# autonomousvision/sdfstudio

Hardware: NVIDIA H100
Metric: rays/sec at 4096 rays x 128 samples (higher is better)
Workload: dtype bf16x3 (fp32 accumulate)

## Files before the change

sdfstudio_b200/csrc/field_tc.h:

```cpp
#pragma once
#include "field_plan.h"

namespace sdfb200 {


constexpr int kEpiWarps = 8;
constexpr int kEpiThreads = kEpiWarps * 32;
constexpr int kTcThreads = kEpiThreads + 128;
constexpr int kEncThreads = 96;
constexpr int kEncItems0 = 288, kEncItems1 = 256, kEncItems2 = 224;
static_assert(kEncItems0 + kEncItems1 + kEncItems2 == 768, "the encoder warps' items cover the tile");
static_assert(kEncItems0 % 32 == 0 && kEncItems1 % 32 == 0, "a warp stages whole 32-row batches (colour_static_tile shuffles across them)");
__host__ __device__ constexpr int enc_item_begin(int w) { return w == 0 ? 0 : w == 1 ? kEncItems0 : w == 2 ? kEncItems0 + kEncItems1 : 768; }
constexpr int kConsumerRegs = 216;
constexpr int kProducerRegs = 72;
static_assert(2 * (kConsumerRegs - 168) <= 168 - kProducerRegs, "setmaxnreg.inc would wait for registers nobody frees");
constexpr int kStages = 5;
constexpr int kKB = 16;
constexpr int kMaxGridDim = 32;
constexpr int kMaxPe = 60;
constexpr int kPeRows = 64;
constexpr int kInK = 96;
constexpr float kHalfPiF = 1.5707963267948966f;
constexpr uint32_t kAPlane = 32 * 2048;
constexpr uint32_t kImgPlane = (kInK / 8) * 128 * 16;
__host__ __device__ constexpr uint32_t tc_stage_bytes(int planes) { return (uint32_t)planes * 256 * kKB * 2; }

enum { PRM_B_G0 = 0, PRM_B_G1, PRM_W_G2 , PRM_B_C0, PRM_B_C1, PRM_W_C2 , kPrmRows = PRM_W_C2 + 3 };
enum { HS_SDF = 0, HS_GRAD , HS_RGB = HS_GRAD + 3 , kHsRows = HS_RGB + 3 };
enum { GEOM_PX = 0, GEOM_PY, GEOM_PZ, GEOM_DX, GEOM_DY, GEOM_DZ, kGeomRows };

struct TcSmem { size_t a, ring, prm, hs, coldesc, hx, bytes; };
__host__ __device__ constexpr TcSmem tc_smem(int planes) {
  TcSmem s{};
  s.ring = s.a + (size_t)planes * kAPlane;
  s.prm = s.ring + (size_t)kStages * tc_stage_bytes(planes);
  s.hs = s.prm + kPrmRows * 256 * 4;
  s.coldesc = s.hs + 2 * kHsRows * 128 * 4;
  s.hx = s.coldesc + 96 * 16;
  s.bytes = s.hx + 128 * 8;
  return s;
}
constexpr size_t kSmemPerBlock = 232448;
constexpr size_t kStaticSmem = 1024;
static_assert(tc_smem(2).bytes + kStaticSmem <= kSmemPerBlock, "shared memory of k_field_tc at two planes");

constexpr size_t kFragWords = 64 * 256;
struct TcScratch { size_t sig, h2, slots, slot_bytes, geo, cs, jpe, jg, geom, ray, bytes; };
__host__ __device__ constexpr TcScratch tc_scratch(int planes) {
  TcScratch s{};
  s.h2 = s.sig + kFragWords * 4;
  s.slots = s.h2 + (size_t)planes * kAPlane;
  s.cs = s.geo + (size_t)planes * kImgPlane;
  s.jpe = s.cs + (size_t)planes * kImgPlane;
  s.jg = s.jpe + (size_t)kPeRows * 128 * 4;
  s.geom = s.jg + (size_t)kMaxGridDim * 3 * 128 * 4;
  s.ray = s.geom + (size_t)kGeomRows * 128 * 4;
  s.slot_bytes = s.ray + 128 * 8;
  s.bytes = s.slots + 2 * s.slot_bytes;
  return s;
}
__host__ __device__ constexpr size_t kScratchPerCta(int planes) { return tc_scratch(planes).bytes; }

__host__ __device__ constexpr int tc_layer_np(int L) { return L == L_B0 ? 128 : 256; }
__host__ __device__ constexpr int tc_layer_k(int L) { return L == L_G0 || L == L_C0MISC ? kInK : 256; }
__host__ __device__ constexpr int tc_layer_kblk(int L) { return kKB * 256 / tc_layer_np(L); }
__host__ __device__ constexpr int tc_layer_nkb(int L) { return tc_layer_k(L) / tc_layer_kblk(L); }
constexpr bool tc_blocks_fill_stages() {
  for (int L = 0; L < L_COUNT; ++L)
    if (tc_layer_np(L) * tc_layer_kblk(L) != 256 * kKB || tc_layer_kblk(L) % 16 != 0 || tc_layer_k(L) % tc_layer_kblk(L) != 0) return false;
  return true;
}
static_assert(tc_blocks_fill_stages(), "every streamed weight block must be one full ring stage of whole K steps");

struct TcLayer {
  unsigned long long w_off;
};

struct TcArgs {
  sdfb200_grid_t grid;
  TcLayer layer[L_COUNT];
  int use_grid, pe_degree, use_pe, contraction, pe_dim, grid_dim, app_dim, use_n_dot_v;
  int mode;
  int n_samples, has_bins, n_tiles;
  long long n_points;
  float rgb_padding, cos_anneal;
  const float *origins, *directions, *bins, *appearance, *variance, *beta, *beta_min;
  const void* table;
  const char* blob;
  unsigned long long b_g0, b_g1, b_g2, w_g2, b_c0, b_c1, w_c2, b_c2;
  char* scratch;
  sdfb200_field_out_t out;
  int render;
  sdfb200_field_render_t rnd;
};

int launch_field_tc_p2_torch(const TcArgs& a, int grid, size_t smem, cudaStream_t st);
int launch_field_tc_p2_tcnn(const TcArgs& a, int grid, size_t smem, cudaStream_t st);
int launch_field_tc_p1_torch(const TcArgs& a, int grid, size_t smem, cudaStream_t st);
int launch_field_tc_p1_tcnn(const TcArgs& a, int grid, size_t smem, cudaStream_t st);

}
```

sdfstudio_b200/csrc/field_tc_kernel.cuh:

```cuda
#pragma once
#include "field_tc.h"
#include "grid.cuh"
#include "tc_common.cuh"

namespace sdfb200 {
using namespace tc;

__device__ __forceinline__ void named_sync(int id, int n) { asm volatile("bar.sync %0, %1;" ::"r"(id), "r"(n) : "memory"); }
constexpr int kEncBar = 3;

__device__ __forceinline__ const float* point_bin(const TcArgs& a, int tile, int row, long long& ray) {
  const long long p0 = (long long)tile * 128;
  const long long ray0 = p0 / a.n_samples;
  const int s = (int)(p0 - ray0 * a.n_samples) + (int)(min(p0 + row, a.n_points - 1) - p0);
  ray = ray0 + s / a.n_samples;
  return a.bins + ray * (a.n_samples + 1) + s % a.n_samples;
}

struct PointGeom { float px, py, pz, dx, dy, dz, delta, t0, t1; long long ray; };
__device__ __forceinline__ PointGeom point_geom(const TcArgs& a, int tile, int row) {
  const long long p = min((long long)tile * 128 + row, a.n_points - 1);
  PointGeom g;
  g.dx = g.dy = g.dz = 0.f; g.delta = 0.f; g.t0 = g.t1 = 0.f;
  g.ray = p;
  if (a.has_bins) {
    const float* bin = point_bin(a, tile, row, g.ray);
    const float t0 = __ldg(bin);
    g.t0 = t0;
    g.t1 = __ldg(bin + 1);
    g.delta = __fsub_rn(g.t1, t0);
    g.dx = __ldg(a.directions + g.ray * 3); g.dy = __ldg(a.directions + g.ray * 3 + 1); g.dz = __ldg(a.directions + g.ray * 3 + 2);
    g.px = __fadd_rn(__ldg(a.origins + g.ray * 3 + 0), __fmul_rn(g.dx, t0));
    g.py = __fadd_rn(__ldg(a.origins + g.ray * 3 + 1), __fmul_rn(g.dy, t0));
    g.pz = __fadd_rn(__ldg(a.origins + g.ray * 3 + 2), __fmul_rn(g.dz, t0));
  } else {
    g.px = __ldg(a.origins + p * 3); g.py = __ldg(a.origins + p * 3 + 1); g.pz = __ldg(a.origins + p * 3 + 2);
    if (a.directions) { g.dx = __ldg(a.directions + p * 3); g.dy = __ldg(a.directions + p * 3 + 1); g.dz = __ldg(a.directions + p * 3 + 2); }
  }
  if (a.contraction != SDFB200_CONTRACT_NONE) {
    const float mag = a.contraction == SDFB200_CONTRACT_LINF
                          ? fmaxf(fabsf(g.px), fmaxf(fabsf(g.py), fabsf(g.pz)))
                          : sqrtf(__fadd_rn(__fadd_rn(__fmul_rn(g.px, g.px), __fmul_rn(g.py, g.py)), __fmul_rn(g.pz, g.pz)));
    if (mag >= 1.f) {
      const float k = __fsub_rn(2.f, __fdiv_rn(1.f, mag));
      g.px = __fmul_rn(k, __fdiv_rn(g.px, mag)); g.py = __fmul_rn(k, __fdiv_rn(g.py, mag)); g.pz = __fmul_rn(k, __fdiv_rn(g.pz, mag));
    }
  }
  return g;
}

static __device__ __forceinline__ void sincos_call(float x, float* s, float* c) { sincosf(x, s, c); }
static __device__ __forceinline__ float sin_call(float x) { return sinf(x); }

template <int P>
struct Slot {
  uint8_t* base;
  __device__ __forceinline__ Slot(char* slots, uint32_t s) : base(reinterpret_cast<uint8_t*>(slots) + s * tc_scratch(P).slot_bytes) {}
  __device__ __forceinline__ uint8_t* geo() const { return base + tc_scratch(P).geo; }
  __device__ __forceinline__ uint8_t* cs() const { return base + tc_scratch(P).cs; }
  __device__ __forceinline__ float* jpe() const { return reinterpret_cast<float*>(base + tc_scratch(P).jpe); }
  __device__ __forceinline__ float* jg() const { return reinterpret_cast<float*>(base + tc_scratch(P).jg); }
  __device__ __forceinline__ float (*geom() const)[128] { return reinterpret_cast<float (*)[128]>(base + tc_scratch(P).geom); }
  __device__ __forceinline__ long long* ray() const { return reinterpret_cast<long long*>(base + tc_scratch(P).ray); }
};

template <int P>
__device__ __forceinline__ void stage_geom(const TcArgs& a, int tile, int et, const Slot<P>& s) {
  float (*gm)[128] = s.geom();
#pragma unroll 1
  for (int row = et; row < 128; row += kEncThreads) {
    const PointGeom g = point_geom(a, tile, row);
    gm[GEOM_PX][row] = g.px; gm[GEOM_PY][row] = g.py; gm[GEOM_PZ][row] = g.pz;
    gm[GEOM_DX][row] = g.dx; gm[GEOM_DY][row] = g.dy; gm[GEOM_DZ][row] = g.dz;
    s.ray()[row] = g.ray;
  }
}

template <int P, int LAYOUT>
__device__ __forceinline__ void encode_tile_grid(const TcArgs& a, int row, int grp, const Slot<P>& s, uint64_t pol_table) {
  const float (*gm)[128] = s.geom();
  float* Jg = s.jg();
  const float x01 = (gm[GEOM_PX][row] + 2.0f) * 0.25f, y01 = (gm[GEOM_PY][row] + 2.0f) * 0.25f, z01 = (gm[GEOM_PZ][row] + 2.0f) * 0.25f;
  const int l_end = min(4 * grp + 4, min(a.grid.n_levels, a.grid.active_levels));
  if (a.use_grid && a.mode != 0) {
#pragma unroll 1
    for (int l = 4 * grp; l < l_end; ++l) {
      LevelCtx c;
      level_prepare<LAYOUT>(a.grid, l, x01, y01, z01, c);
      if (a.grid.table_dtype == SDFB200_DT_F16) level_prefetch_l2<__half, 2>(a.table, c);
      else level_prefetch_l2<float, 2>(a.table, c);
    }
  }
  uint32_t h0 = 0u, h1 = 0u, h2 = 0u, h3 = 0u, l0 = 0u, l1 = 0u, l2 = 0u, l3 = 0u;
#pragma unroll 1
  for (int l = 4 * grp; l < 4 * grp + 4; ++l) {
    float o[2] = {0.f, 0.f};
    float dj[2][3] = {{0.f, 0.f, 0.f}, {0.f, 0.f, 0.f}};
    if (a.use_grid && l < l_end) {
      LevelCtx c;
      float tv[8][2];
      level_prepare<LAYOUT>(a.grid, l, x01, y01, z01, c);
      if (a.grid.table_dtype == SDFB200_DT_F16) level_fetch<__half, 2, true>(a.table, c, tv, pol_table);
      else level_fetch<float, 2, true>(a.table, c, tv, pol_table);
      level_finish<2, LAYOUT>(a.grid, c, tv, o, dj);
    }
    uint32_t hi, lo;
    split2(o[0], o[1], hi, lo);
    h0 = h1; h1 = h2; h2 = h3; h3 = hi;
    l0 = l1; l1 = l2; l2 = l3; l3 = lo;
    if (a.mode != 0 && l < a.grid.n_levels) {
#pragma unroll
      for (int f = 0; f < 2; ++f) {
        const int cg = l * 2 + f;
        Jg[(cg * 3 + 0) * 128 + row] = 0.25f * dj[f][0];
        Jg[(cg * 3 + 1) * 128 + row] = 0.25f * dj[f][1];
        Jg[(cg * 3 + 2) * 128 + row] = 0.25f * dj[f][2];
      }
    }
  }
  store_a_chunk<P>(s.geo(), kImgPlane, row, grp, make_uint4(h0, h1, h2, h3), make_uint4(l0, l1, l2, l3));
}

template <int P>
__device__ __forceinline__ void encode_tile_pe(const TcArgs& a, int tile, int row, const Slot<P>& s) {
  const long long p = (long long)tile * 128 + row;
  const float (*gm)[128] = s.geom();
  const float px = gm[GEOM_PX][row], py = gm[GEOM_PY][row], pz = gm[GEOM_PZ][row];
  if (p < a.n_points) {
    if (a.out.points_norm) a.out.points_norm[p] = sqrtf(__fadd_rn(__fadd_rn(__fmul_rn(px, px), __fmul_rn(py, py)), __fmul_rn(pz, pz)));
    if (a.out.points) { a.out.points[p * 3] = px; a.out.points[p * 3 + 1] = py; a.out.points[p * 3 + 2] = pz; }
  }
  const int deg = a.pe_degree, half = 3 * deg;
  uint8_t* img = s.geo();
  float* Jpe = s.jpe();
  const uint4 z4 = make_uint4(0u, 0u, 0u, 0u);
#pragma unroll 1
  for (int ch = 4; ch < kInK / 8; ++ch) store_a_chunk<P>(img, kImgPlane, row, ch, z4, z4);
#pragma unroll 1
  for (int i = 0; i < a.pe_dim; ++i) {
    const int ia = i >= half ? i - half : i;
    const int b = ia / deg, k = ia - b * deg;
    const float fr = (float)(1 << k);
    const float xb = b == 0 ? px : (b == 1 ? py : pz);
    const float arg = i >= half ? xb * fr + kHalfPiF : xb * fr;
    float sv, cv;
    sincos_call(arg, &sv, &cv);
    store_a<P>(img, kImgPlane, row, 32 + i, a.use_pe ? sv : 0.f);
    if (a.mode != 0) Jpe[i * 128 + row] = a.use_pe ? fr * cv : 0.f;
  }
  store_a<P>(img, kImgPlane, row, 32 + a.pe_dim + 0, px);
  store_a<P>(img, kImgPlane, row, 32 + a.pe_dim + 1, py);
  store_a<P>(img, kImgPlane, row, 32 + a.pe_dim + 2, pz);
}

__device__ __forceinline__ float dir_enc(float dx, float dy, float dz, int k) {
  const int i = k < 12 ? k : k - 12, b = i >> 2;
  const float db = b == 0 ? dx : (b == 1 ? dy : dz);
  const float arg = db * (float)(1 << (i & 3));
  return sin_call(k < 12 ? arg : arg + kHalfPiF);
}

template <int P>
__device__ __forceinline__ void colour_static_tile(const TcArgs& a, int row, const Slot<P>& s) {
  const float (*gm)[128] = s.geom();
  const float px = gm[GEOM_PX][row], py = gm[GEOM_PY][row], pz = gm[GEOM_PZ][row];
  const float dx = gm[GEOM_DX][row], dy = gm[GEOM_DY][row], dz = gm[GEOM_DZ][row];
  const long long ray = s.ray()[row];
  const bool one_ray = __match_any_sync(0xffffffffu, ray) == 0xffffffffu;
  const int lane = row & 31;
  const float own = one_ray && lane < 24 ? dir_enc(dx, dy, dz, lane) : 0.f;
  uint8_t* img = s.cs();
  const uint4 z4 = make_uint4(0u, 0u, 0u, 0u);
#pragma unroll 1
  for (int ch = 1; ch < kInK / 8; ++ch) store_a_chunk<P>(img, kImgPlane, row, ch, z4, z4);
  store_a<P>(img, kImgPlane, row, 8 + 0, px); store_a<P>(img, kImgPlane, row, 8 + 1, py); store_a<P>(img, kImgPlane, row, 8 + 2, pz);
#pragma unroll 1
  for (int k = 0; k < 24; ++k) {
    const float shared = __shfl_sync(0xffffffffu, own, k);
    store_a<P>(img, kImgPlane, row, 8 + 3 + k, one_ray ? shared : dir_enc(dx, dy, dz, k));
  }
  store_a<P>(img, kImgPlane, row, 8 + 27, dx); store_a<P>(img, kImgPlane, row, 8 + 28, dy); store_a<P>(img, kImgPlane, row, 8 + 29, dz);
  if (a.appearance != nullptr) {
#pragma unroll 1
    for (int j = 0; j < a.app_dim; ++j) store_a<P>(img, kImgPlane, row, 8 + 30 + j, __ldg(a.appearance + ray * a.app_dim + j));
  }
}

#ifdef SDFB200_TC_TIMING
__device__ long long g_tc_timing[16 * 48];
#define TC_PUT(tno, k, v)                                                                                            \
  do {                                                                                                               \
    if (blockIdx.x == 0 && (tno) >= 0 && (tno) < 16) g_tc_timing[(tno) * 48 + (k)] = (v);                            \
  } while (0)
#else
#define TC_PUT(tno, k, v) do { (void)(v); } while (0)
#endif
#define TC_STAMP(k) do { if (tid == 0) TC_PUT(tile_no, k, TC_CLOCK()); } while (0)

struct TcBars {
  Handoff<kStages> ring;
  Handoff<2> enc;
  Handoff<1> a;
  Handoff<2> hs;
  uint64_t cop[2][2];
};

template <int P>
__device__ __forceinline__ void produce_all(const TcArgs& a, int nlayers, uint8_t* abuf, uint8_t* ring, char* slots, TcBars& b) {
  uint32_t j = 0;
  int tile_no = 0;
  for (int tile = blockIdx.x; tile < a.n_tiles; tile += gridDim.x, ++tile_no) {
    long long waited = 0;
    b.a.wait_empty(tile_no);
    b.enc.wait_full(tile_no);
    const uint8_t* geo = Slot<P>(slots, b.enc.slot(tile_no)).geo();
    mbar_arrive_expect_tx(b.a.full_bar(tile_no), (uint32_t)P * kImgPlane);
#pragma unroll
    for (int pl = 0; pl < P; ++pl) bulk_g2s(abuf + pl * kAPlane, geo + pl * kImgPlane, kImgPlane, b.a.full_bar(tile_no));
    for (int L = 0; L < nlayers; ++L) {
      for (int kb = 0; kb < tc_layer_nkb(L); ++kb, ++j)
        ring_fill(b.ring, ring, j, reinterpret_cast<const uint8_t*>(a.blob) + a.layer[L].w_off, kb, tc_stage_bytes(P), &waited);
    }
    TC_PUT(tile_no, 10, waited);
  }
}

constexpr int kH2Early = 32 - kInK / 8;
template <int P, int L>
__device__ __forceinline__ void layer_mma(float (&acc)[4][32], bool zero, uint32_t a_base, const uint8_t* ring, Handoff<kStages>& rb, uint32_t& it,
                                          int lane, long long& waited, uint64_t* h2_late, uint32_t h2_parity) {
  constexpr int N = tc_layer_np(L);
  constexpr int KSTEPS = tc_layer_kblk(L) / 16;
  constexpr uint32_t lbo_b = N * 16, plane_b = N * KSTEPS * 16 * 2;
  float (&d)[N / 2] = *reinterpret_cast<float (*)[N / 2]>(&acc[0][0]);
  if (zero) {
#pragma unroll
    for (int i = 0; i < N / 2; ++i) d[i] = 0.f;
  }
#pragma unroll 1
  for (int kb = 0; kb < tc_layer_nkb(L); ++kb, ++it) {
    if (L == L_C0H && kb * KSTEPS == kH2Early / 2) mbar_wait(h2_late, h2_parity);
    rb.wait_full(it, &waited);
    const uint32_t wbase = smem_u32(ring + (size_t)rb.slot(it) * tc_stage_bytes(P));
    wg_fence_acc(d);
    wg_arrive();
#pragma unroll
    for (int j = 0; j < KSTEPS; ++j) {
      const int kstep = kb * KSTEPS + j;
      const int ka = L == L_C0H ? (kstep + kInK / 16) % 16 : kstep;
      wgmma_kstep_wide_ss<P, N>(d, a_desc(a_base, ka), a_desc(a_base + kAPlane, ka), wbase + j * 2 * lbo_b, plane_b, lbo_b);
    }
    wg_commit();
    wg_wait<0>();
    wg_fence_acc(d);
    __syncwarp();
    if (lane == 0) rb.arrive_empty(it);
  }
}

struct TileCtx {
  const TcArgs& a;
  int tid, t, wg, wrow0;
  int r0, cq;
  uint8_t* abuf;
  const float (*prm)[256];
  float (*hs)[128];
  const float4* coldesc;
  float sdf_bias;
  uint32_t* sig_s;
  uint8_t* h2img;
  char* slots;
  __device__ __forceinline__ int unit(int c, int i) const { return (c * 16 + (i >> 1)) * kEpiThreads + tid; }
};

__device__ __forceinline__ uint32_t unorm16x2_encode(float s0, float s1) {
  const float f0 = __fadd_rn(__fmul_rn(s0, 65535.0f), 12582912.0f), f1 = __fadd_rn(__fmul_rn(s1, 65535.0f), 12582912.0f);
  return __byte_perm(__float_as_uint(f0), __float_as_uint(f1), 0x5410);
}
__device__ __forceinline__ float unorm16_lo(uint32_t w) { return __fsub_rn(__uint_as_float(__byte_perm(w, 0x4B00u, 0x5410)), 8388608.0f) * (1.0f / 65535.0f); }
__device__ __forceinline__ float unorm16_hi(uint32_t w) { return __fsub_rn(__uint_as_float(__byte_perm(w, 0x4B00u, 0x5432)), 8388608.0f) * (1.0f / 65535.0f); }

__device__ __forceinline__ void acc_shift(float (&acc)[4][32]) {
#pragma unroll
  for (int c = 0; c < 3; ++c) {
#pragma unroll
    for (int i = 0; i < 32; ++i) acc[c][i] = acc[c + 1][i];
  }
}

template <int N>
__device__ __forceinline__ void load_prm_block(const float* prow, int cq, int c, int j0, float2 (&v)[N]) {
#pragma unroll
  for (int j = 0; j < N; ++j) v[j] = *reinterpret_cast<const float2*>(prow + frag_col(cq, c, 4 * (j0 + j)));
}

template <int P>
__device__ __forceinline__ void epi_e0(const TileCtx& x, float (&acc)[4][32]) {
  const float* p_bg0 = x.prm[PRM_B_G0];
#pragma unroll 1
  for (int c = 0; c < 4; ++c, acc_shift(acc)) {
    float2 bias[8];
    load_prm_block(p_bg0, x.cq, c, 0, bias);
#pragma unroll
    for (int i = 0; i < 32; i += 2) {
      const int col = frag_col(x.cq, c, i), row = frag_row(x.r0, i);
      const float2 b2 = bias[i >> 2];
      float h0, h1, s0, s1;
      softplus100_fast(acc[0][i] + b2.x, h0, s0);
      softplus100_fast(acc[0][i + 1] + b2.y, h1, s1);
      store_a_pair<P>(x.abuf, kAPlane, row, col, h0, h1);
      if (x.a.mode != 0) x.sig_s[x.unit(c, i)] = unorm16x2_encode(s0, s1);
    }
  }
}

template <int P>
__device__ __forceinline__ void epi_e1(const TileCtx& x, int tile, float (&acc)[4][32]) {
  const TcArgs& a = x.a;
  const float* p_bg1 = x.prm[PRM_B_G1];
  const float* p_wg2 = x.prm[PRM_W_G2];
  float sp0 = 0.f, sp1 = 0.f;
#pragma unroll 1
  for (int c = 0; c < 4; ++c, acc_shift(acc)) {
    float2 bias[2], wrow[2];
#pragma unroll
    for (int i = 0; i < 32; i += 2) {
      if (i % 8 == 0) { load_prm_block(p_bg1, x.cq, c, i >> 2, bias); load_prm_block(p_wg2, x.cq, c, i >> 2, wrow); }
      const int col = frag_col(x.cq, c, i), row = frag_row(x.r0, i);
      const float2 b2 = bias[(i >> 2) & 1];
      const float2 w2 = wrow[(i >> 2) & 1];
      float h0, h1, s0, s1;
      softplus100_fast(acc[0][i] + b2.x, h0, s0);
      softplus100_fast(acc[0][i + 1] + b2.y, h1, s1);
      float& sp = frag_half(i) ? sp1 : sp0;
      sp = fmaf(w2.x, h0, sp);
      sp = fmaf(w2.y, h1, sp);
      if (a.mode != 0) {
        store_a_pair<P>(x.h2img, kAPlane, row, col, h0, h1);
        store_a_pair<P>(x.abuf, kAPlane, row, col, w2.x * s0, w2.y * s1);
      }
    }
  }
  if (a.mode != 0) fence_async_global();
  sp0 = quad_sum(sp0);
  sp1 = quad_sum(sp1);
  if ((x.t & 3) < 2) {
    const int h = x.t & 1, row = x.r0 + 8 * h;
    const float sdf = (h ? sp1 : sp0) + x.sdf_bias;
    const long long p = (long long)tile * 128 + row;
    if (p < a.n_points && a.out.sdf) a.out.sdf[p] = sdf;
    if (a.mode != 0) x.hs[HS_SDF][row] = sdf;
  }
}

template <int P>
__device__ __forceinline__ void epi_eb1(const TileCtx& x, float (&acc)[4][32]) {
  uint32_t sw[16], sw_next[16];
#pragma unroll
  for (int k = 0; k < 16; ++k) sw[k] = x.sig_s[x.unit(0, 2 * k)];
#pragma unroll 1
  for (int c = 0; c < 4; ++c, acc_shift(acc)) {
    if (c < 3) {
#pragma unroll
      for (int k = 0; k < 16; ++k) sw_next[k] = x.sig_s[x.unit(c + 1, 2 * k)];
    }
#pragma unroll
    for (int i = 0; i < 32; i += 2) {
      const int col = frag_col(x.cq, c, i), row = frag_row(x.r0, i);
      const uint32_t w = sw[i >> 1];
      store_a_pair<P>(x.abuf, kAPlane, row, col, acc[0][i] * unorm16_lo(w), acc[0][i + 1] * unorm16_hi(w));
    }
    if (c < 3) {
#pragma unroll
      for (int k = 0; k < 16; ++k) sw[k] = sw_next[k];
    }
  }
}

__device__ __forceinline__ float4 col_desc(const TcArgs& a, int ip) {
  const int deg = a.pe_degree, half = 3 * deg;
  int jrow = -1, ax = -1;
  if (ip < a.pe_dim) {
    const int ia = ip >= half ? ip - half : ip;
    ax = ia < deg ? 0 : (ia < 2 * deg ? 1 : 2);
    jrow = ip * 128;
  } else if (ip - a.pe_dim < 3) {
    ax = ip - a.pe_dim;
  }
  return make_float4(__int_as_float(jrow), ax == 0 ? 1.f : 0.f, ax == 1 ? 1.f : 0.f, ax == 2 ? 1.f : 0.f);
}

template <int P>
__device__ __forceinline__ void copy_chunks(uint8_t* abuf, int a_chunk, const uint8_t* src, uint32_t src_plane, int src_chunk, int n, int wrow0,
                                            uint64_t* bar, int lane) {
  for (int k0 = 0; k0 < P * n; k0 += 32) {
    const int k = k0 + lane;
    if (k < P * n) {
      const int pl = k / n, c = k - pl * n;
      bulk_g2s(abuf + pl * kAPlane + (a_chunk + c) * kAChunk + wrow0 * 16, src + pl * src_plane + (src_chunk + c) * kAChunk + wrow0 * 16, 64 * 16, bar);
    }
  }
}
template <int P>
__device__ __forceinline__ void colour_copy(const TileCtx& x, bool early, const uint8_t* cs, uint64_t* bar) {
  constexpr int kMisc = kInK / 8;
  const int lane = x.t & 31;
  if (lane == 0) mbar_arrive_expect_tx(bar, (uint32_t)P * (early ? (kMisc - 1) + kH2Early : 32 - kH2Early) * 64 * 16);
  __syncwarp();
  if (early) {
    copy_chunks<P>(x.abuf, 1, cs, kImgPlane, 1, kMisc - 1, x.wrow0, bar, lane);
    copy_chunks<P>(x.abuf, kMisc, x.h2img, kAPlane, 0, kH2Early, x.wrow0, bar, lane);
  } else {
    copy_chunks<P>(x.abuf, 0, x.h2img, kAPlane, kH2Early, 32 - kH2Early, x.wrow0, bar, lane);
  }
}

template <int P>
__device__ __forceinline__ void epi_eb0(const TileCtx& x, const Slot<P>& s, const float (&acc)[4][32]) {
  const TcArgs& a = x.a;
  const float* Jpe = s.jpe();
  const float* Jg = s.jg();
  float g0x = 0.f, g0y = 0.f, g0z = 0.f, g1x = 0.f, g1y = 0.f, g1z = 0.f;
#pragma unroll
  for (int c = 0; c < 2; ++c) {
#pragma unroll
    for (int i = 0; i < 32; ++i) {
      const int col = frag_col(x.cq, c, i), row = frag_row(x.r0, i);
      const bool h = frag_half(i);
      float& gx = h ? g1x : g0x;
      float& gy = h ? g1y : g0y;
      float& gz = h ? g1z : g0z;
      const float g = acc[c][i];
      if (c == 0 && i < 16) {
        const bool live = col < a.grid_dim;
        const float* j = Jg + col * 3 * 128 + row;
        const float jx = live ? j[0] : 0.f, jy = live ? j[128] : 0.f, jz = live ? j[256] : 0.f;
        gx = fmaf(g, jx, gx); gy = fmaf(g, jy, gy); gz = fmaf(g, jz, gz);
      } else {
        const float4 d = x.coldesc[col - 32];
        const int jrow = __float_as_int(d.x);
        const float tv = __fmul_rn(g, jrow >= 0 ? Jpe[jrow + row] : 1.f);
        gx = fmaf(tv, d.y, gx); gy = fmaf(tv, d.z, gy); gz = fmaf(tv, d.w, gz);
      }
    }
  }
  g0x = quad_sum(g0x); g0y = quad_sum(g0y); g0z = quad_sum(g0z);
  g1x = quad_sum(g1x); g1y = quad_sum(g1y); g1z = quad_sum(g1z);
  if ((x.t & 3) < 2) {
    const int h = x.t & 1, row = x.r0 + 8 * h;
    const float (*gm)[128] = s.geom();
    const float grx = h ? g1x : g0x, gry = h ? g1y : g0y, grz = h ? g1z : g0z;
    const float3 n = normalize_eps(grx, gry, grz);
    const float c0v[8] = {grx, gry, grz, a.use_n_dot_v ? n.x * gm[GEOM_DX][row] + n.y * gm[GEOM_DY][row] + n.z * gm[GEOM_DZ][row] : 0.f,
                          0.f, 0.f, 0.f, 0.f};
    store_a_chunk<P>(x.abuf, kAPlane, row, 0, c0v);
    x.hs[HS_GRAD][row] = grx; x.hs[HS_GRAD + 1][row] = gry; x.hs[HS_GRAD + 2][row] = grz;
  }
}

template <int P>
__device__ __forceinline__ void epi_ec0(const TileCtx& x, float (&acc)[4][32]) {
  const float* p_bc0 = x.prm[PRM_B_C0];
#pragma unroll 1
  for (int c = 0; c < 4; ++c, acc_shift(acc)) {
    float2 bias[8];
    load_prm_block(p_bc0, x.cq, c, 0, bias);
#pragma unroll
    for (int i = 0; i < 32; i += 2) {
      const int col = frag_col(x.cq, c, i), row = frag_row(x.r0, i);
      const float2 b2 = bias[i >> 2];
      store_a_pair<P>(x.abuf, kAPlane, row, col, fmaxf(acc[0][i] + b2.x, 0.f), fmaxf(acc[0][i + 1] + b2.y, 0.f));
    }
  }
}

__device__ __forceinline__ void epi_ec1(const TileCtx& x, float (&acc)[4][32]) {
  const float* p_bc1 = x.prm[PRM_B_C1];
  const float (*p_wc2)[256] = x.prm + PRM_W_C2;
  float r0r = 0.f, r0g = 0.f, r0b = 0.f, r1r = 0.f, r1g = 0.f, r1b = 0.f;
#pragma unroll 1
  for (int c = 0; c < 4; ++c, acc_shift(acc)) {
#pragma unroll
    for (int i = 0; i < 32; ++i) {
      const int col = frag_col(x.cq, c, i);
      const bool h = frag_half(i);
      float& rr = h ? r1r : r0r;
      float& rg = h ? r1g : r0g;
      float& rb = h ? r1b : r0b;
      const float v = fmaxf(acc[0][i] + p_bc1[col], 0.f);
      rr = fmaf(p_wc2[0][col], v, rr);
      rg = fmaf(p_wc2[1][col], v, rg);
      rb = fmaf(p_wc2[2][col], v, rb);
    }
  }
  r0r = quad_sum(r0r); r0g = quad_sum(r0g); r0b = quad_sum(r0b);
  r1r = quad_sum(r1r); r1g = quad_sum(r1g); r1b = quad_sum(r1b);
  if ((x.t & 3) < 2) {
    const int h = x.t & 1, row = x.r0 + 8 * h;
    x.hs[HS_RGB][row] = h ? r1r : r0r; x.hs[HS_RGB + 1][row] = h ? r1g : r0g; x.hs[HS_RGB + 2][row] = h ? r1b : r0b;
  }
}

struct HeadsXfer { double wtot[2][4]; float csum[2][4][8]; };
static_assert(sizeof(TcBars) + sizeof(HeadsXfer) <= kStaticSmem, "static shared memory of k_field_tc (kStaticSmem)");
enum { HR_ALPHA = HS_SDF , HR_NORMAL = HS_GRAD , HR_RGB = HS_RGB  };
struct RayEnd { int q; double tot; float last[3]; };
struct HeadsClock { long long rows, scan, sums; };

__device__ __forceinline__ float sample_mid(const TcArgs& a, int tile, int row) {
  if (!a.has_bins) return 0.f;
  long long ray;
  const float* b = point_bin(a, tile, row, ray);
  return __fdiv_rn(__fadd_rn(__ldg(b), __ldg(b + 1)), 2.0f);
}

__device__ __forceinline__ void heads_rows(const TcArgs& a, float (*hs)[128], double* hx, double* wtot, int tile, int q, int lane,
                                           float& dmin, float& dmax, HeadsClock& clk) {
  long long tc0 = TC_CLOCK();
  const float* b_c2 = reinterpret_cast<const float*>(a.blob + a.b_c2);
  const int row = q * 32 + lane;
  const long long p_raw = (long long)tile * 128 + row;
  const bool valid = p_raw < a.n_points;
  const long long p = valid ? p_raw : a.n_points - 1;
  const PointGeom pg = point_geom(a, tile, row);
  const float dirx = pg.dx, diry = pg.dy, dirz = pg.dz, delta = pg.delta;
  const float sdf = hs[HS_SDF][row], grx = hs[HS_GRAD][row], gry = hs[HS_GRAD + 1][row], grz = hs[HS_GRAD + 2][row];
  const float3 nv = normalize_eps(grx, gry, grz);
  const float nx = nv.x, ny = nv.y, nz = nv.z;
  float rgbv[3];
#pragma unroll
  for (int c = 0; c < 3; ++c) rgbv[c] = padded_rgb(sigmoidf_(hs[HS_RGB + c][row] + __ldg(b_c2 + c)), a.rgb_padding);
  float density = 0.f, alpha = 0.f;
  if (a.out.density || (a.render && a.rnd.from_density)) density = sdf_density(sdf, __ldg(a.beta), __ldg(a.beta_min));
  if (a.out.alpha || (a.render && !a.rnd.from_density))
    alpha = neus_alpha(sdf, dirx * grx + diry * gry + dirz * grz, delta, __ldg(a.variance), a.cos_anneal);
  if (valid) {
    if (a.out.rgb) { a.out.rgb[p * 3] = rgbv[0]; a.out.rgb[p * 3 + 1] = rgbv[1]; a.out.rgb[p * 3 + 2] = rgbv[2]; }
    if (a.out.gradients) { a.out.gradients[p * 3] = grx; a.out.gradients[p * 3 + 1] = gry; a.out.gradients[p * 3 + 2] = grz; }
    if (a.out.normals) { a.out.normals[p * 3] = nx; a.out.normals[p * 3 + 1] = ny; a.out.normals[p * 3 + 2] = nz; }
    if (a.out.density) a.out.density[p] = density;
    if (a.out.occupancy) a.out.occupancy[p] = occupancy(sdf);
    if (a.out.alpha) a.out.alpha[p] = alpha;
  }
  { const long long c = TC_CLOCK(); clk.rows += c - tc0; tc0 = c; }
  if (!a.render) return;
  const int S = a.n_samples;
  const int s_idx = row % S;
  const bool dens = a.rnd.from_density != 0;
  const float dd = valid ? __fmul_rn(delta, density) : 0.f;
  double f = dens ? (double)dd : (valid ? (double)neus_trans_factor(alpha) : 1.0);
  double incl = f;
#pragma unroll
  for (int d = 1; d < 32; d <<= 1) {
    const double o = __shfl_up_sync(0xffffffffu, incl, d);
    if (lane >= d && s_idx >= d) incl = dens ? incl + o : incl * o;
  }
  double excl = __shfl_up_sync(0xffffffffu, incl, 1);
  if (lane == 0 || s_idx == 0) excl = dens ? 0.0 : 1.0;
  const float al = dens ? __fsub_rn(1.0f, expf(-dd)) : alpha;
  const float mid = __fdiv_rn(__fadd_rn(pg.t0, pg.t1), 2.0f);
  if (valid) { dmin = fminf(dmin, mid); dmax = fmaxf(dmax, mid); }
  if (S > 32) {
    if (lane == 31) wtot[q] = incl;
    hx[row] = excl;
    hs[HR_ALPHA][row] = al;
    hs[HR_NORMAL][row] = nx; hs[HR_NORMAL + 1][row] = ny; hs[HR_NORMAL + 2][row] = nz;
    hs[HR_RGB][row] = rgbv[0]; hs[HR_RGB + 1][row] = rgbv[1]; hs[HR_RGB + 2][row] = rgbv[2];
    clk.scan += TC_CLOCK() - tc0;
    return;
  }
  const float T = dens ? expf(-(float)excl) : (float)excl;
  const float w = valid ? __fmul_rn(al, T) : 0.f;
  if (valid && a.rnd.weights) a.rnd.weights[p] = w;
  { const long long c = TC_CLOCK(); clk.scan += c - tc0; tc0 = c; }
  float vs[8] = {w, w * rgbv[0], w * rgbv[1], w * rgbv[2], w * nx, w * ny, w * nz, w * mid};
#pragma unroll
  for (int d = 1; d < 32; d <<= 1) {
    if (d < S) {
#pragma unroll
      for (int k = 0; k < 8; ++k) vs[k] += __shfl_down_sync(0xffffffffu, vs[k], d);
    }
  }
  const int last = (lane - s_idx) + S - 1;
  const double tot = __shfl_sync(0xffffffffu, dens ? excl : incl, last);
  const float lc[3] = {__shfl_sync(0xffffffffu, rgbv[0], last), __shfl_sync(0xffffffffu, rgbv[1], last), __shfl_sync(0xffffffffu, rgbv[2], last)};
  const long long ray = (long long)tile * (128 / S) + row / S;
  if (s_idx == 0 && ray * S < a.n_points) {
    finish_ray(ray, vs[0], {vs[1], vs[2], vs[3]}, {vs[4], vs[5], vs[6]}, vs[7], a.rnd.bg_mode, a.rnd.bg, lc, a.rnd.clamp01, a.rnd.out.rgb,
               a.rnd.out.accumulation, a.rnd.out.normal, a.rnd.out.depth);
    if (a.rnd.bg_transmittance) a.rnd.bg_transmittance[ray] = dens ? expf(-(float)tot) : (float)tot;
  }
  clk.sums += TC_CLOCK() - tc0;
}

__device__ __forceinline__ void composite_chunk(const TcArgs& a, const float (*hs)[128], const double* hx, const double* wtot, float (*csum)[8],
                                                int tile, int q, int lane, RayEnd& end, HeadsClock& clk) {
  long long tc0 = TC_CLOCK();
  const int row = q * 32 + lane;
  const long long p_raw = (long long)tile * 128 + row;
  const bool valid = p_raw < a.n_points;
  const long long p = valid ? p_raw : a.n_points - 1;
  const int S = a.n_samples;
  const bool dens = a.rnd.from_density != 0;
  const int first = (q * 32 / S) * (S / 32);
  double excl = hx[row];
  for (int w2 = first; w2 < q; ++w2) excl = dens ? excl + wtot[w2] : excl * wtot[w2];
  const float T = dens ? expf(-(float)excl) : (float)excl;
  const float w = valid ? __fmul_rn(hs[HR_ALPHA][row], T) : 0.f;
  if (valid && a.rnd.weights) a.rnd.weights[p] = w;
  { const long long c = TC_CLOCK(); clk.scan += c - tc0; tc0 = c; }
  const float rgbv[3] = {hs[HR_RGB][row], hs[HR_RGB + 1][row], hs[HR_RGB + 2][row]};
  float vs[8] = {w, w * rgbv[0], w * rgbv[1], w * rgbv[2], w * hs[HR_NORMAL][row], w * hs[HR_NORMAL + 1][row], w * hs[HR_NORMAL + 2][row],
                 w * sample_mid(a, tile, row)};
#pragma unroll
  for (int d = 1; d < 32; d <<= 1) {
#pragma unroll
    for (int k = 0; k < 8; ++k) vs[k] += __shfl_down_sync(0xffffffffu, vs[k], d);
  }
  if (lane == 0) {
#pragma unroll
    for (int k = 0; k < 8; ++k) csum[q][k] = vs[k];
  }
  if (q == first + S / 32 - 1) {
    end.q = q;
    if (dens) {
      end.tot = __shfl_sync(0xffffffffu, excl, 31);
    } else {
      end.tot = 1.0;
      for (int w2 = first; w2 <= q; ++w2) end.tot *= wtot[w2];
    }
#pragma unroll
    for (int c = 0; c < 3; ++c) end.last[c] = __shfl_sync(0xffffffffu, rgbv[c], 31);
  }
  clk.sums += TC_CLOCK() - tc0;
}

__device__ __forceinline__ void finish_rays(const TcArgs& a, const float (*csum)[8], int tile, int lane, const RayEnd& end, HeadsClock& clk) {
  const long long tc0 = TC_CLOCK();
  const int S = a.n_samples;
  const long long ray = (long long)tile * (128 / S) + end.q * 32 / S;
  if (end.q >= 0 && lane == 0 && ray * S < a.n_points) {
    float s[8] = {0.f, 0.f, 0.f, 0.f, 0.f, 0.f, 0.f, 0.f};
    for (int w2 = end.q + 1 - S / 32; w2 <= end.q; ++w2) {
#pragma unroll
      for (int k = 0; k < 8; ++k) s[k] += csum[w2][k];
    }
    finish_ray(ray, s[0], {s[1], s[2], s[3]}, {s[4], s[5], s[6]}, s[7], a.rnd.bg_mode, a.rnd.bg, end.last, a.rnd.clamp01, a.rnd.out.rgb,
               a.rnd.out.accumulation, a.rnd.out.normal, a.rnd.out.depth);
    const bool dens = a.rnd.from_density != 0;
    if (a.rnd.bg_transmittance) a.rnd.bg_transmittance[ray] = dens ? expf(-(float)end.tot) : (float)end.tot;
  }
  clk.sums += TC_CLOCK() - tc0;
}

__device__ __forceinline__ void heads_of(const TcArgs& a, int tile, int tile_no, int ew, int lane, TcBars& b, float (*hs)[128], double* hx,
                                         HeadsXfer& xf, float& dmin, float& dmax) {
  long long waited = 0, bar_waited = 0;
  b.hs.wait_full(tile_no, &waited);
  const long long t0 = TC_CLOCK();
  float (*h)[128] = hs + b.hs.slot(tile_no) * kHsRows;
  double* wtot = xf.wtot[tile_no & 1];
  float (*csum)[8] = xf.csum[tile_no & 1];
  HeadsClock clk{0, 0, 0};
#pragma unroll 1
  for (int q = ew; q < 4; q += kEncThreads / 32) heads_rows(a, h, hx, wtot, tile, q, lane, dmin, dmax, clk);
  if (a.render && a.n_samples > 32) {
    long long c = TC_CLOCK();
    named_sync(kEncBar, kEncThreads);
    bar_waited += TC_CLOCK() - c;
    RayEnd end{-1, 0.0, {0.f, 0.f, 0.f}};
#pragma unroll 1
    for (int q = ew; q < 4; q += kEncThreads / 32) composite_chunk(a, h, hx, wtot, csum, tile, q, lane, end, clk);
    c = TC_CLOCK();
    named_sync(kEncBar, kEncThreads);
    bar_waited += TC_CLOCK() - c;
    finish_rays(a, csum, tile, lane, end, clk);
  }
  b.hs.arrive_empty(tile_no);
  if (lane == 0) TC_PUT(tile_no, ew == 0 ? 14 : 25 + ew, TC_CLOCK() - t0);
  if (ew == 0 && lane == 0) { TC_PUT(tile_no, 17, waited); TC_PUT(tile_no, 28, clk.rows); TC_PUT(tile_no, 29, clk.scan); TC_PUT(tile_no, 30, clk.sums); TC_PUT(tile_no, 31, bar_waited); }
}

template <int P, int LAYOUT>
__device__ __forceinline__ void encode_all(const TcArgs& a, int ew, int lane, char* slots, TcBars& b, uint64_t pol_table, float (*hs)[128],
                                           double* hx, HeadsXfer& xf) {
  const bool heads = a.mode != 0;
  const int et = ew * 32 + lane;
  const int i_begin = heads ? enc_item_begin(ew) : ew * 32, i_end = heads ? enc_item_begin(ew + 1) : 640, i_step = heads ? 32 : kEncThreads;
  float dmin = INFINITY, dmax = -INFINITY;
  int tile_no = 0;
  for (int tile = blockIdx.x; tile < a.n_tiles; tile += gridDim.x, ++tile_no) {
    long long waited = 0;
    b.enc.wait_empty(tile_no, &waited);
    const long long t0 = TC_CLOCK();
    const Slot<P> s(slots, b.enc.slot(tile_no));
    long long kind_grid = 0, kind_pe = 0, kind_cs = 0, geom = 0;
    stage_geom<P>(a, tile, et, s);
    named_sync(kEncBar, kEncThreads);
    geom = TC_CLOCK() - t0;
#pragma unroll 1
    for (int ib = i_begin; ib < i_end; ib += i_step) {
      const int row = (ib & 127) + lane;
      const long long c0 = TC_CLOCK();
      if (ib < 512) { encode_tile_grid<P, LAYOUT>(a, row, ib >> 7, s, pol_table); kind_grid += TC_CLOCK() - c0; }
      else if (ib < 640) { encode_tile_pe<P>(a, tile, row, s); kind_pe += TC_CLOCK() - c0; }
      else { colour_static_tile<P>(a, row, s); kind_cs += TC_CLOCK() - c0; }
    }
    fence_async_global();
    b.enc.arrive_full(tile_no);
    if (et == 0) { TC_PUT(tile_no, 12, TC_CLOCK() - t0); TC_PUT(tile_no, 13, waited); }
    else if (lane == 0) TC_PUT(tile_no, 23 + ew, TC_CLOCK() - t0);
    if (lane == 0) {
      TC_PUT(tile_no, 32 + 3 * ew, kind_grid); TC_PUT(tile_no, 33 + 3 * ew, kind_pe); TC_PUT(tile_no, 34 + 3 * ew, kind_cs);
      TC_PUT(tile_no, 41 + ew, geom);
    }
    if (heads && tile_no > 0) heads_of(a, tile - (int)gridDim.x, tile_no - 1, ew, lane, b, hs, hx, xf, dmin, dmax);
  }
  if (heads && tile_no > 0) heads_of(a, blockIdx.x + (tile_no - 1) * (int)gridDim.x, tile_no - 1, ew, lane, b, hs, hx, xf, dmin, dmax);
  if (heads && a.render && a.rnd.out.steps_minmax) {
#pragma unroll
    for (int d = 1; d < 32; d <<= 1) {
      dmin = fminf(dmin, __shfl_xor_sync(0xffffffffu, dmin, d));
      dmax = fmaxf(dmax, __shfl_xor_sync(0xffffffffu, dmax, d));
    }
    if (lane == 0 && dmin <= dmax) { atomic_min_float(a.rnd.out.steps_minmax, dmin); atomic_max_float(a.rnd.out.steps_minmax + 1, dmax); }
  }
}

template <int P, int LAYOUT>
__global__ void __launch_bounds__(kTcThreads, 1) k_field_tc(const __grid_constant__ TcArgs a) {
  extern __shared__ __align__(1024) uint8_t smem[];
  constexpr TcSmem sm = tc_smem(P);
  constexpr TcScratch scr = tc_scratch(P);
  uint8_t* abuf = smem + sm.a;
  uint8_t* ring = smem + sm.ring;
  float (*prm)[256] = reinterpret_cast<float (*)[256]>(smem + sm.prm);
  float (*hs)[128] = reinterpret_cast<float (*)[128]>(smem + sm.hs);
  float4* coldesc = reinterpret_cast<float4*>(smem + sm.coldesc);
  double* hx = reinterpret_cast<double*>(smem + sm.hx);
  __shared__ TcBars bars;
  __shared__ HeadsXfer hxf;

  const int tid = threadIdx.x, warp = __shfl_sync(0xffffffffu, tid >> 5, 0), lane = tid & 31;
  const int nlayers = a.mode == 0 ? 2 : L_COUNT;
  char* cta_scr = a.scratch + (size_t)blockIdx.x * scr.bytes;
  char* slots = cta_scr + scr.slots;
  if (tid == 0) {
    bars.ring.init(1, kEpiWarps);
    bars.enc.init(kEncThreads, kEpiThreads);
    bars.hs.init(kEpiThreads, kEncThreads);
    bars.a.init(1, 2);
    for (int w = 0; w < 2; ++w) { mbar_init(&bars.cop[w][0], 1); mbar_init(&bars.cop[w][1], 1); }
    fence_barrier_init();
  }
  {
    const char* blob = a.blob;
    const float* src[kPrmRows] = {reinterpret_cast<const float*>(blob + a.b_g0), reinterpret_cast<const float*>(blob + a.b_g1),
                                  reinterpret_cast<const float*>(blob + a.w_g2), reinterpret_cast<const float*>(blob + a.b_c0),
                                  reinterpret_cast<const float*>(blob + a.b_c1), reinterpret_cast<const float*>(blob + a.w_c2),
                                  reinterpret_cast<const float*>(blob + a.w_c2) + 256, reinterpret_cast<const float*>(blob + a.w_c2) + 512};
    for (int i = tid; i < kPrmRows * 256; i += kTcThreads) prm[i >> 8][i & 255] = src[i >> 8][i & 255];
    if (tid < 96) coldesc[tid] = col_desc(a, tid);
  }
  __syncthreads();

  constexpr int kEncWarp0 = (kTcThreads - kEncThreads) / 32;
  if (warp >= kEpiWarps) {
    setmaxnreg_dec<kProducerRegs>();
    if (warp == kEpiWarps) {
      if (lane == 0) produce_all<P>(a, nlayers, abuf, ring, slots, bars);
    } else if (warp >= kEncWarp0) {
      encode_all<P, LAYOUT>(a, warp - kEncWarp0, lane, slots, bars, l2_policy_evict_last(), hs, hx, hxf);
    }
    return;
  }
  setmaxnreg_inc<kConsumerRegs>();

  const int wg = warp >> 2, t = tid & 127;
  const int wrow0 = wg * 64;
  const int wg_bar = 1 + wg;
  const uint32_t a_base = smem_u32(abuf) + wrow0 * 16;
  const float sdf_bias = __ldg(reinterpret_cast<const float*>(a.blob + a.b_g2));
  TileCtx x{a, tid, t, wg, wrow0, frag_row0(wrow0, t), frag_cq(t), abuf, prm, hs, coldesc, sdf_bias,
            reinterpret_cast<uint32_t*>(cta_scr + scr.sig), reinterpret_cast<uint8_t*>(cta_scr + scr.h2), slots};
  uint32_t it = 0;
  long long waited = 0;
  float acc[4][32];
#define SYNC_A()                \
  do {                          \
    fence_async_smem();         \
    named_sync(wg_bar, 128);    \
  } while (0)
#define LAYER(L, zero)                                                                                 \
  do {                                                                                                 \
    layer_mma<P, L>(acc, zero, a_base, ring, bars.ring, it, lane, waited, &bars.cop[wg][1], tile_no & 1); \
    named_sync(wg_bar, 128);   \
    TC_STAMP(1 + (L));                                                                                 \
  } while (0)

  int tile_no = -1;
  for (int tile = blockIdx.x; tile < a.n_tiles; tile += gridDim.x) {
    ++tile_no;
    TC_STAMP(0);
    waited = 0;
    const Slot<P> s(slots, bars.enc.slot(tile_no));
    x.hs = hs + bars.hs.slot(tile_no) * kHsRows;
    bars.a.wait_full(tile_no);
    if (a.mode == 0) bars.enc.arrive_empty(tile_no);
    TC_STAMP(8);
    LAYER(L_G0, true);
    epi_e0<P>(x, acc);
    TC_STAMP(18);
    SYNC_A();
    LAYER(L_G1, true);
    if (a.mode == 0) {
      if (t == 0) bars.a.arrive_empty(tile_no);
      epi_e1<P>(x, tile, acc);
      continue;
    }
    {
      long long hs_waited = 0;
      bars.hs.wait_empty(tile_no, &hs_waited);
      if (tid == 0) TC_PUT(tile_no, 16, hs_waited);
    }
    epi_e1<P>(x, tile, acc);
    TC_STAMP(19);
    SYNC_A();
    LAYER(L_B1, true);
    epi_eb1<P>(x, acc);
    TC_STAMP(20);
    SYNC_A();
    LAYER(L_B0, true);
    bars.enc.wait_full(tile_no);
    if ((warp & 3) == 0) colour_copy<P>(x, true, s.cs(), &bars.cop[wg][0]);
    epi_eb0<P>(x, s, acc);
    mbar_wait(&bars.cop[wg][0], tile_no & 1);
    bars.enc.arrive_empty(tile_no);
    TC_STAMP(21);
    SYNC_A();
    LAYER(L_C0MISC, true);
    if ((warp & 3) == 0) colour_copy<P>(x, false, nullptr, &bars.cop[wg][1]);
    TC_STAMP(22);
    LAYER(L_C0H, false);
    epi_ec0<P>(x, acc);
    TC_STAMP(23);
    SYNC_A();
    LAYER(L_C1, true);
    if (t == 0) bars.a.arrive_empty(tile_no);
    epi_ec1(x, acc);
    bars.hs.arrive_full(tile_no);
    TC_STAMP(15);
    if (tid == 0) TC_PUT(tile_no, 9, waited);
  }
#undef SYNC_A
#undef LAYER
}

template <int P, int LAYOUT>
static int launch_field_tc(const TcArgs& a, int grid, size_t smem, cudaStream_t st) {
  SDFB_CUDA(cudaFuncSetAttribute(k_field_tc<P, LAYOUT>, cudaFuncAttributeMaxDynamicSharedMemorySize, (int)smem));
  k_field_tc<P, LAYOUT><<<grid, kTcThreads, smem, st>>>(a);
  SDFB_LAUNCHED("k_field_tc");
  return 0;
}

}
```

sdfstudio_b200/csrc/grid.cuh:

```cuda
#pragma once
#include "common.cuh"

namespace sdfb200 {

constexpr uint32_t kPrimeY = 2654435761u;
constexpr uint32_t kPrimeZ = 805459861u;

__device__ __forceinline__ uint64_t l2_policy_evict_last() {
  uint64_t p;
  asm volatile("createpolicy.fractional.L2::evict_last.b64 %0, 1.0;" : "=l"(p));
  return p;
}

template <typename T, int F, bool HINT = false>
__device__ __forceinline__ void load_row(const void* table, uint64_t row, float (&v)[F], uint64_t pol = 0) {
  const T* p = reinterpret_cast<const T*>(table) + row * F;
  if constexpr (HINT) {
    static_assert(F == 2, "hinted loads are only used by the F=2 fused kernel");
    if constexpr (sizeof(T) == 4) {
      asm volatile("ld.global.nc.L2::cache_hint.v2.f32 {%0, %1}, [%2], %3;" : "=f"(v[0]), "=f"(v[1]) : "l"(p), "l"(pol));
    } else {
      uint32_t raw;
      asm volatile("ld.global.nc.L2::cache_hint.b32 %0, [%1], %2;" : "=r"(raw) : "l"(p), "l"(pol));
      const float2 t = __half22float2(*reinterpret_cast<const __half2*>(&raw));
      v[0] = t.x; v[1] = t.y;
    }
  } else if constexpr (sizeof(T) == 4) {
    if constexpr (F == 1) {
      v[0] = __ldg(p);
    } else if constexpr (F == 2) {
      float2 t = __ldg(reinterpret_cast<const float2*>(p));
      v[0] = t.x; v[1] = t.y;
    } else {
#pragma unroll
      for (int i = 0; i < F; i += 4) {
        float4 t = __ldg(reinterpret_cast<const float4*>(p + i));
        v[i] = t.x; v[i + 1] = t.y; v[i + 2] = t.z; v[i + 3] = t.w;
      }
    }
  } else {
    if constexpr (F == 1) {
      v[0] = __half2float(p[0]);
    } else if constexpr (F == 2) {
      float2 t = __half22float2(__ldg(reinterpret_cast<const __half2*>(p)));
      v[0] = t.x; v[1] = t.y;
    } else if constexpr (F == 4) {
      uint2 raw = __ldg(reinterpret_cast<const uint2*>(p));
      float2 a = __half22float2(*reinterpret_cast<__half2*>(&raw.x));
      float2 b = __half22float2(*reinterpret_cast<__half2*>(&raw.y));
      v[0] = a.x; v[1] = a.y; v[2] = b.x; v[3] = b.y;
    } else {
#pragma unroll
      for (int i = 0; i < F; i += 8) {
        uint4 raw = __ldg(reinterpret_cast<const uint4*>(p + i));
        const __half2* h = reinterpret_cast<const __half2*>(&raw);
#pragma unroll
        for (int j = 0; j < 4; ++j) {
          float2 a = __half22float2(h[j]);
          v[i + 2 * j] = a.x; v[i + 2 * j + 1] = a.y;
        }
      }
    }
  }
}

template <int LAYOUT>
__device__ __forceinline__ bool torch_layout(const sdfb200_grid_t& g) {
  return LAYOUT < 0 ? g.layout == SDFB200_GRID_TORCH : LAYOUT == SDFB200_GRID_TORCH;
}

struct LevelCtx {
  uint32_t idx[8];
  uint64_t base;
  float w[3], dw[3], d2w[3], s;
};

template <int LAYOUT = -1>
__device__ __forceinline__ void level_prepare(const sdfb200_grid_t& g, int l, float x, float y, float z, LevelCtx& c) {
  if constexpr (LAYOUT < 0) {
    if (g.layout == SDFB200_GRID_TORCH) level_prepare<SDFB200_GRID_TORCH>(g, l, x, y, z, c);
    else level_prepare<SDFB200_GRID_TCNN>(g, l, x, y, z, c);
    return;
  }
  constexpr bool torch = LAYOUT == SDFB200_GRID_TORCH;
  const float s = g.scale[l];
  const float xs[3] = {x, y, z};
  uint32_t lo[3], hi[3];
  c.s = s;
  c.base = g.offset[l];
#pragma unroll
  for (int d = 0; d < 3; ++d) {
    const float p = torch ? __fmul_rn(xs[d], s) : fmaf(xs[d], s, 0.5f);
    const float fl = floorf(p);
    lo[d] = (uint32_t)(int)fl;
    hi[d] = torch ? (uint32_t)(int)ceilf(p) : lo[d] + 1u;
    const float t = __fsub_rn(p, fl);
    if (g.smoothstep) {
      c.w[d] = __fmul_rn(__fmul_rn(t, t), __fsub_rn(3.0f, __fmul_rn(2.0f, t)));
      c.dw[d] = 6.f * t * (1.f - t);
      c.d2w[d] = (6.f - 12.f * t) * s * s;
    } else {
      c.w[d] = t; c.dw[d] = 1.f; c.d2w[d] = 0.f;
    }
  }
  const uint32_t mask = (1u << g.log2_hashmap_size) - 1u;
#pragma unroll
  for (int k = 0; k < 8; ++k) {
    const uint32_t ix = (k & 1) ? hi[0] : lo[0], iy = (k & 2) ? hi[1] : lo[1], iz = (k & 4) ? hi[2] : lo[2];
    const uint32_t h = ix ^ (iy * kPrimeY) ^ (iz * kPrimeZ);
    if (torch) {
      c.idx[k] = h & mask;
    } else {
      const uint32_t res = g.resolution[l];
      c.idx[k] = (g.hashed[l] ? h : ix + iy * res + iz * res * res) % g.size[l];
    }
  }
}

template <typename T, int F, bool HINT = false>
__device__ __forceinline__ void level_fetch(const void* table, const LevelCtx& c, float (&v)[8][F], uint64_t pol = 0) {
#pragma unroll
  for (int k = 0; k < 8; ++k) load_row<T, F, HINT>(table, c.base + c.idx[k], v[k], pol);
}

template <typename T, int F>
__device__ __forceinline__ void level_prefetch_l2(const void* table, const LevelCtx& c) {
#pragma unroll
  for (int k = 0; k < 8; ++k)
    asm volatile("prefetch.global.L2::evict_last [%0];" ::"l"(reinterpret_cast<const T*>(table) + (c.base + c.idx[k]) * F));
}

template <int F, int LAYOUT = -1>
__device__ __forceinline__ void level_finish(const sdfb200_grid_t& g, const LevelCtx& c, const float (&v)[8][F], float (&out)[F], float (&dout)[F][3]) {
  if (torch_layout<LAYOUT>(g)) {
    const float(&f0)[F] = v[7], (&f1)[F] = v[5], (&f2)[F] = v[4], (&f3)[F] = v[6], (&f4)[F] = v[3], (&f5)[F] = v[1], (&f6)[F] = v[0], (&f7)[F] = v[2];
    const float ox = c.w[0], oy = c.w[1], oz = c.w[2];
    const float nx = __fsub_rn(1.f, ox), ny = __fsub_rn(1.f, oy), nz = __fsub_rn(1.f, oz);
#pragma unroll
    for (int f = 0; f < F; ++f) {
      const float f03 = __fadd_rn(__fmul_rn(f0[f], ox), __fmul_rn(f3[f], nx));
      const float f12 = __fadd_rn(__fmul_rn(f1[f], ox), __fmul_rn(f2[f], nx));
      const float f56 = __fadd_rn(__fmul_rn(f5[f], ox), __fmul_rn(f6[f], nx));
      const float f47 = __fadd_rn(__fmul_rn(f4[f], ox), __fmul_rn(f7[f], nx));
      const float f0312 = __fadd_rn(__fmul_rn(f03, oy), __fmul_rn(f12, ny));
      const float f4756 = __fadd_rn(__fmul_rn(f47, oy), __fmul_rn(f56, ny));
      out[f] = __fadd_rn(__fmul_rn(f0312, oz), __fmul_rn(f4756, nz));
      const float gx = ((f0[f] - f3[f]) * oy + (f1[f] - f2[f]) * ny) * oz + ((f4[f] - f7[f]) * oy + (f5[f] - f6[f]) * ny) * nz;
      const float gy = (f03 - f12) * oz + (f47 - f56) * nz;
      const float gz = f0312 - f4756;
      dout[f][0] = gx * c.dw[0] * c.s; dout[f][1] = gy * c.dw[1] * c.s; dout[f][2] = gz * c.dw[2] * c.s;
    }
  } else {
#pragma unroll
    for (int f = 0; f < F; ++f) { out[f] = 0.f; dout[f][0] = dout[f][1] = dout[f][2] = 0.f; }
#pragma unroll
    for (int k = 0; k < 8; ++k) {
      const float wx = (k & 1) ? c.w[0] : 1.f - c.w[0], wy = (k & 2) ? c.w[1] : 1.f - c.w[1], wz = (k & 4) ? c.w[2] : 1.f - c.w[2];
      const float wt = wx * wy * wz;
#pragma unroll
      for (int f = 0; f < F; ++f) {
        out[f] = fmaf(wt, v[k][f], out[f]);
        dout[f][0] += ((k & 1) ? 1.f : -1.f) * wy * wz * v[k][f];
        dout[f][1] += ((k & 2) ? 1.f : -1.f) * wx * wz * v[k][f];
        dout[f][2] += ((k & 4) ? 1.f : -1.f) * wx * wy * v[k][f];
      }
    }
#pragma unroll
    for (int f = 0; f < F; ++f) { dout[f][0] *= c.dw[0] * c.s; dout[f][1] *= c.dw[1] * c.s; dout[f][2] *= c.dw[2] * c.s; }
  }
}

template <typename T, int F>
__device__ __forceinline__ void encode_level(const sdfb200_grid_t& g, const void* table, int l, float x, float y, float z,
                                             float (&out)[F], float (&dout)[F][3]) {
  LevelCtx c;
  float v[8][F];
  level_prepare(g, l, x, y, z, c);
  level_fetch<T, F>(table, c, v);
  level_finish<F>(g, c, v, out, dout);
}

__device__ __forceinline__ void corner_weights(const LevelCtx& c, float (&w)[8]) {
#pragma unroll
  for (int k = 0; k < 8; ++k)
    w[k] = ((k & 1) ? c.w[0] : 1.f - c.w[0]) * ((k & 2) ? c.w[1] : 1.f - c.w[1]) * ((k & 4) ? c.w[2] : 1.f - c.w[2]);
}

}
```

Baseline: 1.540 million.

## Rebalance encoder warp items, restructure PE loop, drop evict_last prefetch hint

Moves the encoder warp item split from 288/256/224 to 256/224/288 and adds a rotation offset for the 'heads' path so each warp's work mix changes. The positional-encoding loop now iterates per axis with a doubling frequency, computing the sin and shifted-cos pair in one iteration, which removes the per-element integer divides. It also zero-fills only the A-image chunks past the PE data. Separately, the L2 prefetch of hash-table rows no longer uses the evict_last policy, which may change L2 retention of the table.

```diff
diff --git a/sdfstudio_b200/csrc/field_tc.h b/sdfstudio_b200/csrc/field_tc.h
--- a/sdfstudio_b200/csrc/field_tc.h
+++ b/sdfstudio_b200/csrc/field_tc.h
@@ -8,9 +8,11 @@
 constexpr int kEpiThreads = kEpiWarps * 32;
 constexpr int kTcThreads = kEpiThreads + 128;
 constexpr int kEncThreads = 96;
-constexpr int kEncItems0 = 288, kEncItems1 = 256, kEncItems2 = 224;
+constexpr int kEncItems0 = 256, kEncItems1 = 224, kEncItems2 = 768 - 256 - 224;
+constexpr int kEncItemShift = 32;
 static_assert(kEncItems0 + kEncItems1 + kEncItems2 == 768, "the encoder warps' items cover the tile");
-static_assert(kEncItems0 % 32 == 0 && kEncItems1 % 32 == 0, "a warp stages whole 32-row batches (colour_static_tile shuffles across them)");
+static_assert(kEncItems0 % 32 == 0 && kEncItems1 % 32 == 0 && kEncItemShift % 32 == 0,
+              "a warp stages whole 32-row batches of one kind (colour_static_tile shuffles across them)");
 __host__ __device__ constexpr int enc_item_begin(int w) { return w == 0 ? 0 : w == 1 ? kEncItems0 : w == 2 ? kEncItems0 + kEncItems1 : 768; }
 constexpr int kConsumerRegs = 216;
 constexpr int kProducerRegs = 72;
diff --git a/sdfstudio_b200/csrc/field_tc_kernel.cuh b/sdfstudio_b200/csrc/field_tc_kernel.cuh
--- a/sdfstudio_b200/csrc/field_tc_kernel.cuh
+++ b/sdfstudio_b200/csrc/field_tc_kernel.cuh
@@ -135,18 +135,22 @@
   float* Jpe = s.jpe();
   const uint4 z4 = make_uint4(0u, 0u, 0u, 0u);
 #pragma unroll 1
-  for (int ch = 4; ch < kInK / 8; ++ch) store_a_chunk<P>(img, kImgPlane, row, ch, z4, z4);
-#pragma unroll 1
-  for (int i = 0; i < a.pe_dim; ++i) {
-    const int ia = i >= half ? i - half : i;
-    const int b = ia / deg, k = ia - b * deg;
-    const float fr = (float)(1 << k);
-    const float xb = b == 0 ? px : (b == 1 ? py : pz);
-    const float arg = i >= half ? xb * fr + kHalfPiF : xb * fr;
-    float sv, cv;
-    sincos_call(arg, &sv, &cv);
-    store_a<P>(img, kImgPlane, row, 32 + i, a.use_pe ? sv : 0.f);
-    if (a.mode != 0) Jpe[i * 128 + row] = a.use_pe ? fr * cv : 0.f;
+  for (int ch = (32 + a.pe_dim + 3) / 8; ch < kInK / 8; ++ch) store_a_chunk<P>(img, kImgPlane, row, ch, z4, z4);
+#pragma unroll 1
+  for (int b = 0; b < 3; ++b) {
+    const float xb = gm[GEOM_PX + b][row];
+    float fr = 1.f;
+#pragma unroll 1
+    for (int i = b * deg; i < b * deg + deg; ++i, fr *= 2.f) {
+      const float arg = xb * fr;
+      float sv, cv;
+      sincos_call(arg, &sv, &cv);
+      store_a<P>(img, kImgPlane, row, 32 + i, a.use_pe ? sv : 0.f);
+      if (a.mode != 0) Jpe[i * 128 + row] = a.use_pe ? fr * cv : 0.f;
+      sincos_call(arg + kHalfPiF, &sv, &cv);
+      store_a<P>(img, kImgPlane, row, 32 + half + i, a.use_pe ? sv : 0.f);
+      if (a.mode != 0) Jpe[(half + i) * 128 + row] = a.use_pe ? fr * cv : 0.f;
+    }
   }
   store_a<P>(img, kImgPlane, row, 32 + a.pe_dim + 0, px);
   store_a<P>(img, kImgPlane, row, 32 + a.pe_dim + 1, py);
@@ -700,10 +704,11 @@
     geom = TC_CLOCK() - t0;
 #pragma unroll 1
     for (int ib = i_begin; ib < i_end; ib += i_step) {
-      const int row = (ib & 127) + lane;
+      const int it = heads ? (ib + kEncItemShift) % 768 : ib;
+      const int row = (it & 127) + lane;
       const long long c0 = TC_CLOCK();
-      if (ib < 512) { encode_tile_grid<P, LAYOUT>(a, row, ib >> 7, s, pol_table); kind_grid += TC_CLOCK() - c0; }
-      else if (ib < 640) { encode_tile_pe<P>(a, tile, row, s); kind_pe += TC_CLOCK() - c0; }
+      if (it < 512) { encode_tile_grid<P, LAYOUT>(a, row, it >> 7, s, pol_table); kind_grid += TC_CLOCK() - c0; }
+      else if (it < 640) { encode_tile_pe<P>(a, tile, row, s); kind_pe += TC_CLOCK() - c0; }
       else { colour_static_tile<P>(a, row, s); kind_cs += TC_CLOCK() - c0; }
     }
     fence_async_global();
diff --git a/sdfstudio_b200/csrc/grid.cuh b/sdfstudio_b200/csrc/grid.cuh
--- a/sdfstudio_b200/csrc/grid.cuh
+++ b/sdfstudio_b200/csrc/grid.cuh
@@ -127,7 +127,7 @@
 __device__ __forceinline__ void level_prefetch_l2(const void* table, const LevelCtx& c) {
 #pragma unroll
   for (int k = 0; k < 8; ++k)
-    asm volatile("prefetch.global.L2::evict_last [%0];" ::"l"(reinterpret_cast<const T*>(table) + (c.base + c.idx[k]) * F));
+    asm volatile("prefetch.global.L2 [%0];" ::"l"(reinterpret_cast<const T*>(table) + (c.base + c.idx[k]) * F));
 }
 
 template <int F, int LAYOUT = -1>
```

After: 1.547 million (median of 6 runs). Within noise of the previous version (+0.5%).
